# KinWaiCheuk/ReconVAT

Hardware: AMD Instinct MI355X
Metric: training audio-sec/sec (node) (higher is better)
Workload: dtype f32; 1 GPU; ReconVAT UNet_Onset VAT=True reconstruction=True, per-GPU B_l=8 + B_ul=8 segments of 327680 samples (640 frames x 229 mel), Adam+StepLR, fp32; parallelism=dp1, hipgraph=True, two_stream_schedule=True, kernel_plan_table=644fe159bb9eb70e, kernel_plan_mode=table, vat_nan_flag=0

## Files before the change

### include/reconvat_hip.h

```cpp
#ifndef RECONVAT_HIP_H
#define RECONVAT_HIP_H

#ifdef __cplusplus
extern "C" {
#endif

int rv_abi_version(void);
const char* rv_last_error(void);
const char* rv_source_digest(void);

int rv_melspec_lognorm_fwd(const float* audio, long audio_stride, int B, int nsamp, const float* window,
                           const float* twiddle, const int* mel_start, const int* mel_len, const float* mel_w, int mel_ld,
                           int n_mels, int hop, int do_log, int normalise, float* out, int T, void* workspace, void* stream);

long rv_cqt_workspace_bytes(int B, int nsamp, int n_items, int hop, int kernel_width);
int rv_cqt_lognorm_fwd(const float* audio, long audio_stride, int B, int nsamp, const float* w, long w_floats, const int* items,
                       int n_items, const int* groups, int n_groups, const float* scale, int n_bins, int kernel_width, int hop,
                       int do_log, int normalise, float* out, int T, void* workspace, long workspace_bytes, void* stream);

long rv_packed_weight_floats(int taps, int kdim, int ndim);
int rv_pack_weights(const float* w, float* out, int taps, int kdim, int ndim, long s_k, long s_n, int flip,
                    int scatter_cmid, int force_plain, void* stream);
long rv_pack_table_entry_bytes(void);
long rv_pack_table_fill(void* table_host, int i, const float* w, float* out, int taps, int kdim, int ndim, long s_k, long s_n,
                        int flip, int scatter_cmid, int force_plain);
int rv_pack_table_run(const void* table_dev, int count, long total_blocks, void* stream);
int rv_conv_fwd(int mode, const float* in, int in_ld, int B, int H, int W, int Cin, float* out, int out_ld, int Ho,
                int Wo, int Cout, const float* wpack, const float* bias, int accumulate, int algo, double* bn_sums,
                const float* bn_z, int bn_z_ld, const float* bn_coef, float bn_slope, void* stream);
long rv_conv_wgrad_workspace_bytes(int taps, int B, int Hv, int Ca, int Cb);
int rv_conv_wgrad_set_plan(int taps, int B, int Hv, int Ca, int Cb, int nw, int wgs);
int rv_conv_wgrad(int mode, const float* U, int u_ld, int Hu, int Wu, int Ca, const float* V, int v_ld, int Hv, int Wv,
                  int Cb, int B, float* dw, long s_a, long s_b, int flip, float* dbias, int accumulate, void* workspace,
                  long workspace_bytes, void* stream);
long rv_conv_wgrad_deferred(int mode, const float* U, int u_ld, int Hu, int Wu, int Ca, const float* V, int v_ld, int Hv, int Wv,
                            int Cb, int B, float* dw, long s_a, long s_b, int flip, float* dbias, void* workspace,
                            long workspace_bytes, void* entry_host, void* stream);
int rv_conv_wgrad_seg(int mode, int nseg, const float* const* U, const float* const* V, int u_ld, int Hu, int Wu, int Ca, int v_ld, int Hv,
                      int Wv, int Cb, int Bseg, float* dw, long s_a, long s_b, int flip, float* dbias, int accumulate, void* workspace,
                      long workspace_bytes, void* stream);
long rv_conv_wgrad_deferred_seg(int mode, int nseg, const float* const* U, const float* const* V, int u_ld, int Hu, int Wu, int Ca, int v_ld,
                                int Hv, int Wv, int Cb, int Bseg, float* dw, long s_a, long s_b, int flip, float* dbias, void* workspace,
                                long workspace_bytes, void* entry_host, void* stream);
long rv_wgrad_table_entry_bytes(void);
long rv_wgrad_table_finalize(void* table_host, int count);
int rv_wgrad_reduce_table(const void* table_dev, int count, long total_blocks, void* stream);


long rv_bn_workspace_bytes(int C);
int rv_bn_lrelu_fwd(const float* z, int z_ld, long P, int C, const float* gamma, const float* beta, float* running_mean,
                    float* running_var, long* num_batches_tracked, float momentum, float eps, int training, float slope,
                    const float* res, int res_ld, float* y, int y_ld, float* coef, void* workspace, int sums_ready,
                    void* stream);
int rv_bn_lrelu_fwd_skip(const float* z, int z_ld, long P, int C, const float* gamma, const float* beta, float* running_mean,
                         float* running_var, long* num_batches_tracked, float momentum, float eps, int training, float slope,
                         const float* x, int x_ld, int cin, const float* w, const float* b, int ksplit, float* y, int y_ld, float* coef,
                         void* workspace, int sums_ready, void* stream);
int rv_bn_running_update(float* running_mean, float* running_var, long* num_batches_tracked, const float* coef, int C,
                         float momentum, void* stream);
int rv_bn_running_update_table(const long* table, int nlayers, float momentum, void* stream);
int rv_bn_lrelu_bwd(const float* dy, int dy_ld, const float* z, int z_ld, long P, int C, const float* coef, float slope,
                    int frozen, float* dz, int dz_ld, float* dgamma, float* dbeta, int param_accumulate, void* workspace,
                    int sums_ready, void* stream);

long rv_gemm_splitk_workspace_bytes(int M, int N, int splitk, int batch);
long rv_gemm_splitk_ticket_bytes(int M, int N, int splitk, int batch);
int rv_gemm(const float* A, long sam, long sak, const float* B, long sbk, long sbn, float* C, long scm, long scn, float* C2,
            long sc2m, long sc2n, const float* bias, int M, int N, int K, int act, int accumulate, int splitk, int batch,
            long bsa, long bsb, long bsc, float* a_rowsum, void* splitk_ws, void* splitk_tickets, void* stream);
long rv_gemm_table_entry_bytes(void);
long rv_gemm_table_fill(void* entry_host, const float* A, long sam, long sak, const float* B, long sbk, long sbn, float* C, long scm,
                        long scn, const float* bias, int M, int N, int K, int splitk, int batch, long bsa, long bsb, long bsc,
                        float* a_rowsum, void* splitk_ws);
long rv_gemm_table_finalize(void* table_host, int count, long* fold_blocks);
int rv_gemm_table_run(const void* table_dev, int count, long total_blocks, long fold_blocks, int orientation, void* stream);
int rv_sigmoid_bwd(const float* g1, int ld1, const float* g2, int ld2, const float* y, int ldy, float* dz, int ldz, long M,
                   int N, void* stream);
int rv_colsum(const float* x, int ld, long M, int N, float* out, int accumulate, void* stream);
long rv_colsum_ordered_workspace_bytes(long M, int N);
int rv_colsum_ordered(const float* x, int ld, long M, int N, float* out, int accumulate, void* ws, void* stream);
int rv_sums_fold(const double* sums, int C, int c0, int n, float* out, int accumulate, void* stream);

// ... 82 lines not shown
```

### reconvat_amd/_lib.py

```python
import ctypes
import os

import torch

_HERE = os.path.dirname(os.path.abspath(__file__))
LIB_PATH = os.environ.get('RECONVAT_HIP_LIB') or os.path.join(_HERE, 'libreconvat_hip.so')

P = ctypes.c_void_p
U = ctypes.c_uint
I = ctypes.c_int
L = ctypes.c_long
F = ctypes.c_float

SIGNATURES = {
    'rv_abi_version': (I, []),
    'rv_last_error': (ctypes.c_char_p, []),
    'rv_source_digest': (ctypes.c_char_p, []),
    'rv_melspec_lognorm_fwd': (I, [P, L, I, I, P, P, P, P, P, I, I, I, I, I, P, I, P, P]),
    'rv_cqt_workspace_bytes': (L, [I, I, I, I, I]),
    'rv_cqt_lognorm_fwd': (I, [P, L, I, I, P, L, P, I, P, I, P, I, I, I, I, I, P, I, P, L, P]),
    'rv_packed_weight_floats': (L, [I, I, I]),
    'rv_pack_weights': (I, [P, P, I, I, I, L, L, I, I, I, P]),
    'rv_pack_table_entry_bytes': (L, []),
    'rv_pack_table_fill': (L, [P, I, P, P, I, I, I, L, L, I, I, I]),
    'rv_pack_table_run': (I, [P, I, L, P]),
    'rv_conv_fwd': (I, [I, P, I, I, I, I, I, P, I, I, I, I, P, P, I, I, P, P, I, P, F, P]),
    'rv_conv_wgrad_workspace_bytes': (L, [I, I, I, I, I]),
    'rv_conv_wgrad_set_plan': (I, [I, I, I, I, I, I, I]),
    'rv_conv_wgrad': (I, [I, P, I, I, I, I, P, I, I, I, I, I, P, L, L, I, P, I, P, L, P]),
    'rv_conv_wgrad_deferred': (L, [I, P, I, I, I, I, P, I, I, I, I, I, P, L, L, I, P, P, L, P, P]),
    'rv_conv_wgrad_seg': (I, [I, I, P, P, I, I, I, I, I, I, I, I, I, P, L, L, I, P, I, P, L, P]),
    'rv_conv_wgrad_deferred_seg': (L, [I, I, P, P, I, I, I, I, I, I, I, I, I, P, L, L, I, P, P, L, P, P]),
    'rv_wgrad_table_entry_bytes': (L, []),
    'rv_wgrad_table_finalize': (L, [P, I]),
    'rv_wgrad_reduce_table': (I, [P, I, L, P]),
    'rv_bn_workspace_bytes': (L, [I]),
    'rv_bn_lrelu_fwd': (I, [P, I, L, I, P, P, P, P, P, F, F, I, F, P, I, P, I, P, P, I, P]),
    'rv_bn_lrelu_fwd_skip': (I, [P, I, L, I, P, P, P, P, P, F, F, I, F, P, I, I, P, P, I, P, I, P, P, I, P]),
    'rv_bn_running_update': (I, [P, P, P, P, I, F, P]),
    'rv_bn_running_update_table': (I, [P, I, F, P]),
    'rv_bn_lrelu_bwd': (I, [P, I, P, I, L, I, P, F, I, P, I, P, P, I, P, I, P]),
    'rv_gemm_splitk_workspace_bytes': (L, [I, I, I, I]),
    'rv_gemm_splitk_ticket_bytes': (L, [I, I, I, I]),
    'rv_gemm': (I, [P, L, L, P, L, L, P, L, L, P, L, L, P, I, I, I, I, I, I, I, L, L, L, P, P, P, P]),
    'rv_gemm_table_entry_bytes': (L, []),
    'rv_gemm_table_fill': (L, [P, P, L, L, P, L, L, P, L, L, P, I, I, I, I, I, L, L, L, P, P]),
    'rv_gemm_table_finalize': (L, [P, I, P]),
    'rv_gemm_table_run': (I, [P, I, L, L, I, P]),
    'rv_sigmoid_bwd': (I, [P, I, P, I, P, I, P, I, L, I, P]),
    'rv_colsum': (I, [P, I, L, I, P, I, P]),
    'rv_colsum_ordered_workspace_bytes': (L, [L, I]),
    'rv_colsum_ordered': (I, [P, I, L, I, P, I, P, P]),
    'rv_sums_fold': (I, [P, I, I, I, P, I, P]),
    'rv_local_attn_fwd': (I, [P, P, P, L, P, P, P, I, I, I, I, P]),
    'rv_local_attn_bwd': (I, [P, P, P, P, L, P, P, P, P, P, L, P, I, I, I, I, P]),
    'rv_vat_perturb_fwd': (I, [P, P, L, I, F, F, P, P, P, P, P]),
    'rv_vat_perturb_bwd': (I, [P, P, P, L, I, F, F, P, P]),
    'rv_reduce_workspace_bytes': (L, [L]),
    'rv_reduce_mean': (I, [I, P, P, L, P, P, P, P]),
    'rv_loss_bwd': (I, [I, P, P, L, P, P, P]),
    'rv_adam_step': (I, [P, P, P, P, L, P, F, L, F, F, F, F, F, P, P]),
    'rv_counter_add': (I, [P, L, P, P]),
    'rv_clip_scale': (I, [P, L, P, F, P]),
    'rv_adamw_step': (I, [P, P, P, P, L, P, F, L, F, F, F, F, F, P, F, F, P, P, F, P]),
    'rv_swap_floats': (I, [P, P, L, P]),
    'rv_crop_segments': (I, [P, P, P, P, P, I, L, I, I, P, P, P, P, P, P]),
    'rv_crop_segments_shift': (I, [P, L, P, P, L, P, L, P, I, L, I, I, P, P, P, P, P, P]),
    'rv_fir_items': (I, [P, L, P, I, I, P, P, I, L, P, L, P]),
    'rv_resample_max_coeffs': (L, []),
    'rv_resample': (I, [P, I, L, I, L, P, I, I, I, I, P, I, L, L, P]),
    'rv_eval_workspace_bytes': (L, [L]),
    'rv_eval_decode': (I, [P, P, L, F, F, I, P, L, P, P, P, L, P]),
    'rv_eval_decode_clean': (I, [P, P, L, F, F, I, I, I, P, L, P, P, P, L, P]),
    'rv_eval_frame_counts': (I, [P, P, L, P, P, L, P]),
    'rv_eval_sweep_workspace_bytes': (L, [L, I, I]),
    'rv_eval_sweep': (I, [P, P, L, P, I, P, I, I, P, L, P, P, P, P, L, P]),
    'rv_eval_sweep_clean': (I, [P, P, L, P, I, P, I, I, I, I, P, L, P, P, P, P, L, P]),
    'rv_lstm_flag_bytes': (L, [I]),
    'rv_lstm_fwd': (I, [P, P, P, P, P, P, P, P, I, I, I, P]),
# ... 74 lines not shown
```

### reconvat_amd/csrc/conv.hip

```cpp
#include "conv_band.h"
#include <mutex>

struct PackArgs {
    const float* w;
    float* out;
    int taps, kdim, ndim;
    int R, ntile_n, nchunk;
    long s_k, s_n;
    int flip;
    int scatter_cmid;
    long total;
    long wino0;
};

__device__ __forceinline__ void pack_wino_elem(const PackArgs& a, long idx) {
    const int R = a.R;
    int r = (int)(idx % R);
    long t = idx / R;
    int lane = (int)(t % 64); t /= 64;
    int nt = (int)(t % a.ntile_n); t /= a.ntile_n;
    int c = (int)(t % a.nchunk);
    int xi = (int)(t / a.nchunk);
    int k = c * 4 * R + (lane >> 4) * R + r;
    int n = nt * 16 + (lane & 15);
// ... 174 lines not shown
#pragma unroll
            for (int n = 0; n < NT; ++n) {
                const int q = m * NT + n;
                if (q % KS != wave) continue;
                f32x4 sum = part[0][q][lane];
#pragma unroll
                for (int w = 1; w < KS; ++w) sum += part[w][q][lane];
                acc[m][n] = sum;
            }
    }
    f32x4 bv[NT];
#pragma unroll
    for (int n = 0; n < NT; ++n) {
        const int ncol = (nt0 + n) * 16 + 4 * g;
        const int cb = SCATTER ? ncol % a.Cout : ncol;
#pragma unroll
        for (int r = 0; r < 4; ++r) bv[n][r] = (a.bias && cb + r < a.Cout) ? a.bias[cb + r] : 0.f;
    }
#pragma unroll
    for (int m = 0; m < MT; ++m) {
        if (!pv[m]) continue;
#pragma unroll
        for (int n = 0; n < NT; ++n) {
            if (KS > 1 && (m * NT + n) % KS != wave) continue;
            const int ncol = (nt0 + n) * 16 + 4 * g;
            int co0;
            long opix;
            bool inside = true;
            if (SCATTER) {
                const int tap4 = ncol / a.Cout;
                co0 = ncol - tap4 * a.Cout;
                const int oy = py[m] * 2 + (tap4 >> 1), ox = px[m] * 2 + (tap4 & 1);
                inside = tap4 < 4 && oy < a.Ho && ox < a.Wo;
                opix = ((long)pb[m] * a.Ho + oy) * a.Wo + ox;
            } else {
                co0 = ncol;
                opix = (tile0 + m) * 16 + j;
            }
            if (!inside || co0 >= a.Cout) continue;
            float* o = a.out + opix * a.out_ld + co0;
            f32x4 v = acc[m][n] + bv[n];
            if (a.vec_store && co0 + 3 < a.Cout) {
                if (a.accumulate) {
                    f32x4 old = *reinterpret_cast<f32x4*>(o);
                    v += old;
                }
                *reinterpret_cast<f32x4*>(o) = v;
            } else {
#pragma unroll
                for (int r = 0; r < 4; ++r)
                    if (co0 + r < a.Cout) o[r] = a.accumulate ? o[r] + v[r] : v[r];
            }
        }
    }
}

__device__ __attribute__((aligned(16))) const float rv_zero_piece[256] = {0.f};

typedef short s16x4 __attribute__((ext_vector_type(4)));
typedef __bf16 bf16x2_t __attribute__((ext_vector_type(2)));
typedef __bf16 bf16x4_t __attribute__((ext_vector_type(4)));
__device__ __forceinline__ s16x4 to_bf16x4(const f32x4& v) {
    const bf16x2_t lo = __builtin_convertvector((f32x2){v[0], v[1]}, bf16x2_t);
    const bf16x2_t hi = __builtin_convertvector((f32x2){v[2], v[3]}, bf16x2_t);
    const bf16x4_t q = __builtin_shufflevector(lo, hi, 0, 1, 2, 3);
    return __builtin_bit_cast(s16x4, q);
}

template <int R, int NT, int MTW, int NW, bool BF = false>
__global__ __launch_bounds__(NW * 64) void conv3x3_lds_k(ConvLdsArgs aa) {
    static_assert(!BF || R == 4, "the bf16 path needs 16-channel chunks");
    constexpr int NTHR = NW * 64;
    typedef typename VecR<R>::T vec;
    constexpr int KC = 4 * R;
    constexpr int Q = R;
    constexpr int PPI = 64 / Q;
    constexpr int LPF = 16 * R;
    constexpr int FPI = 64 / LPF;
    constexpr int WFLOATS = 9 * NT * 64 * R;
    const ConvArgs& a = aa.c;
    extern __shared__ __attribute__((aligned(16))) float smem[];
    const int tid = threadIdx.x, lane = tid & 63;
    const int wave = __builtin_amdgcn_readfirstlane(tid >> 6);
    const int j = lane & 15, g = lane >> 4;
    const int W = a.W, H = a.H, W2 = W + 2, TH = aa.TH;
    const int nrow = TH + 2;
    const int xfloats = nrow * W2 * KC;
    if (ABL(aa) & 32) return;
    const int vid = aa.xcd ? xcd_remap(blockIdx.x, gridDim.x) : blockIdx.x;
    const int grp = vid / aa.nsplit, split = vid - grp * aa.nsplit;
    const int nt0 = split * NT;
    const int nbuf = aa.nbuf;
    float* xs0 = smem;
    float* ws0 = smem + nbuf * xfloats;
    const int band_lo = grp * aa.bands_per_wg;
    const int band_hi = min(band_lo + aa.bands_per_wg, aa.total_bands);
    if (band_lo >= band_hi) return;
    const int nchunk = a.nchunk;
    const int nunits = (band_hi - band_lo) * nchunk;
    const int ipr = (W + PPI - 1) / PPI;

    constexpr int TXF = 4;
    constexpr int NWF = (9 * NT + FPI - 1) / FPI;
    constexpr int TW = (NWF + NW - 1) / NW;
    const int nx = nrow * ipr;
    int xs_row[TXF], xs_ldst[TXF];
// ... 2047 lines not shown
        ent = tab[lo];
    }
    __syncthreads();
    const long block = (long)blockIdx.x - ent.block0;
#ifdef RV_ABLATION
    if (plain) {
        ent.a.accumulate = 0;
        if (ent.vec4 && ent.el == 64) wgrad_reduce_body_v4<64, false>(ent.a, block, sh);
        else if (ent.vec4 && ent.el == 16) wgrad_reduce_body_v4<16, false>(ent.a, block, sh);
        else if (ent.el == 64) wgrad_reduce_body<64, false>(ent.a, block, sh);
        else if (ent.el == 16) wgrad_reduce_body<16, false>(ent.a, block, sh);
        else wgrad_reduce_body<4, false>(ent.a, block, sh);
        return;
    }
#endif
    if (ent.vec4 && ent.el == 1024) wgrad_reduce_body_v4<1024, true>(ent.a, block, sh);
    else if (ent.vec4 && ent.el == 64) wgrad_reduce_body_v4<64, true>(ent.a, block, sh);
    else if (ent.vec4 && ent.el == 16) wgrad_reduce_body_v4<16, true>(ent.a, block, sh);
    else if (ent.el == 64) wgrad_reduce_body<64, true>(ent.a, block, sh);
    else if (ent.el == 16) wgrad_reduce_body<16, true>(ent.a, block, sh);
    else wgrad_reduce_body<4, true>(ent.a, block, sh);
}

template <int KH, int KW, int S, int P, int R, bool SC>
static int launch_conv_rt(const ConvArgs& a, int NT, int MT, hipStream_t st, bool ksplit = false) {
    const long ntiles = (a.npix + 15) / 16;
    if (ksplit) {
        if constexpr (R == 4 && !(KH == 3)) {
#define RV_CASEK(nt, mt)                                                                         \
    if (NT == nt && MT == mt) {                                                                  \
        dim3 grid(cdiv(ntiles, mt), a.ntile_n / nt);                                             \
        hipLaunchKernelGGL((conv_mfma_k<KH, KW, S, P, R, nt, mt, SC, 4>), grid, dim3(256), 0, st, a); \
        return RV_OK;                                                                            \
    }
            RV_CASEK(1, 1) RV_CASEK(1, 2) RV_CASEK(2, 1) RV_CASEK(2, 2) RV_CASEK(1, 4) RV_CASEK(4, 1)
#undef RV_CASEK
        }
        return RV_EUNSUPPORTED;
    }
#define RV_CASE(nt, mt)                                                                          \
    if (NT == nt && MT == mt) {                                                                  \
        dim3 grid(cdiv(ntiles, 4 * mt), a.ntile_n / nt);                                         \
        hipLaunchKernelGGL((conv_mfma_k<KH, KW, S, P, R, nt, mt, SC>), grid, dim3(256), 0, st, a); \
        return RV_OK;                                                                            \
    }
    RV_CASE(1, 1) RV_CASE(1, 2) RV_CASE(1, 4)
    RV_CASE(2, 1) RV_CASE(2, 2) RV_CASE(2, 4)
    RV_CASE(3, 1) RV_CASE(3, 2) RV_CASE(3, 4)
    RV_CASE(4, 1) RV_CASE(4, 2) RV_CASE(4, 4)
#undef RV_CASE
    return RV_EUNSUPPORTED;
}

static void choose_tiles(long ntiles, int ntile_n, int* NT, int* MT) {
    static const int nts[4] = {4, 3, 2, 1};
    static const int mts[3] = {4, 2, 1};
    int best_nt = 1, best_mt = 1;
    long best_score = -1;
    for (int a = 0; a < 4; ++a) {
        int nt = nts[a];
        if (ntile_n % nt) continue;
        for (int b = 0; b < 3; ++b) {
            int mt = mts[b];
            long waves = ((ntiles + mt - 1) / mt) * (ntile_n / nt);
            long reuse = (long)(nt * mt * 100) / (nt + mt);
            long fill = waves >= 2048 ? 100 : (waves * 100) / 2048;
            long score = reuse * fill;
            if (score > best_score) { best_score = score; best_nt = nt; best_mt = mt; }
        }
    }
    *NT = best_nt; *MT = best_mt;
}

static size_t conv3x3_lds_bytes(int R, int NT, int TH, int W, int nchunk, int nbuf = 2) {
    return ((size_t)nbuf * (TH + 2) * (W + 2) * 4 * R + (size_t)(nchunk > 1 ? nbuf : 1) * 9 * NT * 64 * R) * sizeof(float);
}

template <int R, int NW, bool BF = false>
static int launch_conv3x3_lds_r(const ConvArgs& a, int NT, int MTW, int TH, int wgs_per_cu, hipStream_t st) {
    ConvLdsArgs aa;
    aa.c = a; aa.TH = TH;
    dim3 grid(band_grid(aa, NT, 256 * wgs_per_cu)), blk(NW * 64);
    static const int nbuf_env = getenv("RV_CONV_NBUF") ? atoi(getenv("RV_CONV_NBUF")) : 0;
    aa.nbuf = 2;
    if (nbuf_env == 3 && conv3x3_lds_bytes(R, NT, TH, a.W, a.nchunk, 3) <= (size_t)(wgs_per_cu > 1 ? 76 : 150) * 1024) aa.nbuf = 3;
    aa.ablate = getenv("RV_ABLATE") ? atoi(getenv("RV_ABLATE")) : 0;
    static const int skew_env = getenv("RV_CONV_SKEW") ? atoi(getenv("RV_CONV_SKEW")) : 1;
    aa.skew = (aa.nbuf == 3 && NW >= 8) ? skew_env : 0;
    const size_t lds = conv3x3_lds_bytes(R, NT, TH, a.W, a.nchunk, aa.nbuf);
#define RV_L3(nt, mt)                                                                              \
    if (NT == nt && MTW == mt) {                                                                  \
        auto kern = conv3x3_lds_k<R, nt, mt, NW, BF>;                                             \
         \
        static std::once_flag attr_once;                                                          \
        std::call_once(attr_once, [&] {                                                           \
             \
            if (hipFuncSetAttribute((const void*)kern, hipFuncAttributeMaxDynamicSharedMemorySize, 156 * 1024) != hipSuccess) \
                (void)hipGetLastError();                                                          \
        });                                                                                       \
        hipLaunchKernelGGL(kern, grid, blk, lds, st, aa);                                         \
        return RV_OK;                                                                             \
    }
    if constexpr (NW == 12) {
        RV_L3(1, 3) RV_L3(2, 3) RV_L3(3, 3) RV_L3(4, 3)
        RV_L3(1, 5) RV_L3(2, 5) RV_L3(1, 6) RV_L3(2, 6)
        RV_L3(1, 1) RV_L3(2, 1) RV_L3(4, 1) RV_L3(1, 2) RV_L3(2, 2) RV_L3(4, 2) RV_L3(1, 4) RV_L3(2, 4)
// ... 149 lines not shown
    }
    return RV_OK;
}

int rv_pack_weights(const float* w, float* out, int taps, int kdim, int ndim, long s_k, long s_n, int flip,
                    int scatter_cmid, int force_plain, void* stream) {
    PackArgs a;
    const int rc = pack_args_make(a, w, out, taps, kdim, ndim, s_k, s_n, flip, scatter_cmid, force_plain);
    if (rc != RV_OK) return rc;
    hipStream_t st = (hipStream_t)stream;
    if (a.R == 0) hipLaunchKernelGGL(pack_plain_k, dim3(cdiv(a.total, 256)), dim3(256), 0, st, a);
    else hipLaunchKernelGGL(pack_frag_k, dim3(cdiv(a.total, 256)), dim3(256), 0, st, a);
    RV_LAUNCH_CHECK("rv_pack_weights");
    return RV_OK;
}

long rv_pack_table_entry_bytes(void) { return (long)sizeof(PackEntry); }

long rv_pack_table_fill(void* table, int i, const float* w, float* out, int taps, int kdim, int ndim, long s_k, long s_n,
                        int flip, int scatter_cmid, int force_plain) {
    PackEntry* tab = (PackEntry*)table;
    if (pack_args_make(tab[i].a, w, out, taps, kdim, ndim, s_k, s_n, flip, scatter_cmid, force_plain) != RV_OK) return -1;
    tab[i].block0 = i == 0 ? 0 : tab[i - 1].block0 + cdiv(tab[i - 1].a.total, 256);
    return tab[i].block0 + cdiv(tab[i].a.total, 256);
}

int rv_pack_table_run(const void* table_dev, int count, long total_blocks, void* stream) {
    RV_CHECK_ARG(count > 0 && total_blocks > 0 && total_blocks < (1L << 31), "rv_pack_table_run: empty or oversized table");
    hipLaunchKernelGGL(pack_table_k, dim3((unsigned)total_blocks), dim3(256), 0, (hipStream_t)stream,
                       (const PackEntry*)table_dev, count);
    RV_LAUNCH_CHECK("rv_pack_table_run");
    return RV_OK;
}

struct BnFuse { double* sums; const float* z; int z_ld; const float* coef; float slope; };
static int conv_fwd_impl(int mode, const float* in, int in_ld, int B, int H, int W, int Cin, float* out, int out_ld, int Ho,
                         int Wo, int Cout, const float* wpack, const float* bias, int accumulate, int algo, const BnFuse& bn,
                         bool* sums_done, hipStream_t st);

int rv_conv_fwd(int mode, const float* in, int in_ld, int B, int H, int W, int Cin, float* out, int out_ld, int Ho,
                int Wo, int Cout, const float* wpack, const float* bias, int accumulate, int algo, double* bn_sums,
                const float* bn_z, int bn_z_ld, const float* bn_coef, float bn_slope, void* stream) {
    hipStream_t st = (hipStream_t)stream;
    bool sums_done = false;
    RV_CHECK_ARG(!bn_z || (bn_sums && bn_coef), "rv_conv_fwd: bn_z needs bn_sums and bn_coef");
    const BnFuse bn = {bn_sums, bn_z, bn_z_ld, bn_coef, bn_slope};
    const int rc = conv_fwd_impl(mode, in, in_ld, B, H, W, Cin, out, out_ld, Ho, Wo, Cout, wpack, bias, accumulate, algo,
                                 bn, &sums_done, st);
    if (rc != RV_OK || !bn_sums || sums_done) return rc;
    if (bn_z) return rv_internal_bn_bwd_stats(out, out_ld, bn_z, bn_z_ld, (long)B * Ho * Wo, Cout, bn_coef, bn_slope, bn_sums, st);
    return rv_internal_bn_stats(out, out_ld, (long)B * Ho * Wo, Cout, bn_sums, st);
}

static int conv_fwd_impl(int mode, const float* in, int in_ld, int B, int H, int W, int Cin, float* out, int out_ld, int Ho,
                         int Wo, int Cout, const float* wpack, const float* bias, int accumulate, int algo, const BnFuse& bn,
                         bool* sums_done, hipStream_t st) {
    double* bn_sums = bn.sums;
    RV_CHECK_ARG(mode >= 0 && mode <= 3, "rv_conv_fwd: bad mode %d", mode);
    if (mode == 0 || mode == 1) RV_CHECK_ARG(Ho == H && Wo == W, "rv_conv_fwd: same-size conv needs Ho==H, Wo==W");
    if (mode == 2) RV_CHECK_ARG(Ho == H / 2 && Wo == W / 2, "rv_conv_fwd: down conv needs Ho=H/2, Wo=W/2");
    if (mode == 3)
        RV_CHECK_ARG(Ho >= 2 * H && Ho <= 2 * H + 1 && Wo >= 2 * W && Wo <= 2 * W + 1,
                     "rv_conv_fwd: up conv needs 2H<=Ho<=2H+1 (got H=%d Ho=%d W=%d Wo=%d)", H, Ho, W, Wo);
    const int R = frag_R(Cin);
    const bool small = (R == 0) || (Cout <= 2 && mode != 3);
    if (small) {
        SmallArgs s;
        s.in = in; s.in_ld = in_ld; s.H = H; s.W = W; s.out = out; s.out_ld = out_ld; s.Ho = Ho; s.Wo = Wo;
        s.B = B; s.wplain = wpack; s.bias = bias; s.npix = (long)B * Ho * Wo; s.accumulate = accumulate;
        s.fd_plane = fastdiv_make((unsigned)(Ho * Wo)); s.fd_wo = fastdiv_make((unsigned)Wo);
        const int tpp = Cout / small_cpt(Cin, Cout, mode == 0 ? 9 : 1);
        RV_CHECK_ARG(s.npix * tpp < (1L << 31), "rv_conv_fwd: more than 2^31 outputs");
        s.bn_sums = (Cout >= 4 && !bn.z) ? bn_sums : nullptr;
        if (s.bn_sums) *sums_done = true;
        long nblk = cdiv(s.npix * tpp, 256);
        const long cap = s.bn_sums ? 1024 : 4096;
        if (nblk > cap) nblk = cap;
        dim3 grid((unsigned)nblk), blk(256);
#define RV_SMALL(ci, co, kh, kw, ss, pp)                                                          \
    if (Cin == ci && Cout == co) {                                                               \
        hipLaunchKernelGGL((conv_small_k<ci, co, kh, kw, ss, pp>), grid, blk, 0, st, s);         \
        RV_LAUNCH_CHECK("conv_small");                                                           \
        return RV_OK;                                                                            \
    }
#define RV_NARROW(ci, co)                                                                         \
    if (mode == 0 && Cin == ci && Cout == co && (in_ld & 3) == 0 && ((((uintptr_t)in) & 15) == 0)) { \
        RV_CHECK_ARG(s.npix < (1L << 28), "rv_conv_fwd: more than 2^28 pixels");                \
        static const int nrows_env = getenv("RV_NARROW_ROWS") ? atoi(getenv("RV_NARROW_ROWS")) : 16;   \
        s.rows = nrows_env;                                                                      \
        const long nb = (long)B * cdiv(H, s.rows) * cdiv(W, 256 / (ci / 4));                     \
        hipLaunchKernelGGL((conv_narrow_out_k<ci, co>), dim3((unsigned)nb), blk, 0, st, s);      \
        RV_LAUNCH_CHECK("conv_narrow_out");                                                      \
        return RV_OK;                                                                            \
    }
        RV_NARROW(16, 1) RV_NARROW(8, 2) RV_NARROW(8, 1)
#undef RV_NARROW
        static const int cin1_env = getenv("RV_CONV_CIN1") ? atoi(getenv("RV_CONV_CIN1")) : 1;
        const bool cin12 = mode == 0 && ((Cin == 1 && (Cout == 16 || Cout == 8)) || (Cin == 2 && Cout == 8 && (in_ld & 1) == 0 && ((((uintptr_t)in) & 7) == 0)));
        const bool bz_ok = !bn.z || ((bn.z_ld & 3) == 0 && ((((uintptr_t)bn.z) & 15) == 0) && ((((uintptr_t)bn.coef) & 15) == 0));
        if (cin1_env && cin12 && bz_ok && (!bias || ((((uintptr_t)bias) & 15) == 0))) {
            s.rows = 16;
            s.bn_z = bn.z; s.bn_z_ld = bn.z_ld; s.bn_coef = bn.coef; s.bn_slope = bn.slope;
            if (bn.z) { s.bn_sums = bn_sums; *sums_done = true; }
            const long nb = (long)B * cdiv(H, s.rows) * cdiv(W, 1024 / Cout);
            if (Cin == 1 && Cout == 16) hipLaunchKernelGGL((conv_cin12_k<1, 16>), dim3((unsigned)nb), blk, 0, st, s);
            else if (Cin == 1) hipLaunchKernelGGL((conv_cin12_k<1, 8>), dim3((unsigned)nb), blk, 0, st, s);
            else hipLaunchKernelGGL((conv_cin12_k<2, 8>), dim3((unsigned)nb), blk, 0, st, s);
            RV_LAUNCH_CHECK("conv_cin12");
            return RV_OK;
        }
        if (mode == 0) {
            RV_SMALL(1, 16, 3, 3, 1, 1) RV_SMALL(16, 1, 3, 3, 1, 1)
            RV_SMALL(8, 2, 3, 3, 1, 1)  RV_SMALL(2, 8, 3, 3, 1, 1)
            RV_SMALL(8, 1, 3, 3, 1, 1)  RV_SMALL(1, 8, 3, 3, 1, 1)
            RV_SMALL(1, 48, 3, 3, 1, 1) RV_SMALL(48, 1, 3, 3, 1, 1)
        } else if (mode == 1) {
            RV_SMALL(1, 16, 1, 1, 1, 0) RV_SMALL(16, 1, 1, 1, 1, 0)
        }
#undef RV_SMALL
        rv_set_error("rv_conv_fwd: no small-channel kernel for mode %d Cin=%d Cout=%d", mode, Cin, Cout);
        return RV_EUNSUPPORTED;
    }
    ConvArgs a;
    a.in = in; a.in_ld = in_ld; a.H = H; a.W = W; a.out = out; a.out_ld = out_ld; a.Ho = Ho; a.Wo = Wo;
    a.B = B; a.Cin = Cin; a.Cout = Cout; a.wpack = wpack; a.bias = bias; a.bn_sums = bn_sums;
    a.bn_z = bn.z; a.bn_z_ld = bn.z_ld; a.bn_coef = bn.coef; a.bn_slope = bn.slope;
    a.nchunk = Cin / (4 * R);
    a.accumulate = accumulate;
    a.vec_store = ((out_ld & 3) == 0) && ((((uintptr_t)out) & 15) == 0);
    RV_CHECK_ARG((in_ld % R) == 0 && ((((uintptr_t)in) & (4 * R - 1)) == 0), "rv_conv_fwd: input not %d-byte aligned", 4 * R);
    if (mode == 3) {
        RV_CHECK_ARG(Cout % 16 == 0, "rv_conv_fwd: scatter conv needs Cout %% 16 == 0");
        a.ntile_n = 4 * Cout / 16;
        a.Ph = H + (Ho - 2 * H); a.Pw = W + (Wo - 2 * W);
    } else {
        a.ntile_n = (Cout + 15) / 16;
        a.Ph = Ho; a.Pw = Wo;
    }
    a.npix = (long)B * a.Ph * a.Pw;
    a.fd_pw = fastdiv_make((unsigned)a.Pw); a.fd_plane = fastdiv_make((unsigned)(a.Ph * a.Pw)); a.fd_w = fastdiv_make((unsigned)W);
    RV_CHECK_ARG(a.npix < (1L << 31), "rv_conv_fwd: more than 2^31 pixels");
    const bool bf = ((algo >> 20) & 1) && mode == 0 && R == 4;
    algo &= ~(1 << 20);
    const int fam = (algo >> 8) & 15, f_nt = (algo >> 4) & 15, f_mt = algo & 15, f_th = (algo >> 12) & 255;
    if (fam == 6 || fam == 10 || fam == 12) {
        if (mode != 0 || R != 4) { rv_set_error("rv_conv_fwd: the Winograd kernel needs a 3x3 conv with Cin %% 16 == 0"); return RV_EUNSUPPORTED; }
        const int rcw = fam == 6 ? launch_conv3x3_wino<8>(a, f_nt, f_mt, f_th, st)
                                 : (fam == 10 ? launch_conv3x3_wino<8, true>(a, f_nt, f_mt, f_th, st) : launch_conv3x3_wino<12, true>(a, f_nt, f_mt, f_th, st));
        if (rcw != RV_OK) { rv_set_error("rv_conv_fwd: forced Winograd tile NT=%d MTW=%d TH=%d does not fit", f_nt, f_mt, f_th); return rcw; }
        RV_LAUNCH_CHECK("rv_conv_fwd(winograd)");
        *sums_done = true;
        return RV_OK;
    }
    if (fam == 14) {
        if (mode != 0 || R != 4) { rv_set_error("rv_conv_fwd: the Winograd kernel needs a 3x3 conv with Cin %% 16 == 0"); return RV_EUNSUPPORTED; }
        const int rcw = launch_conv3x3_wino<4, true>(a, f_nt, f_mt, f_th, st, (size_t)78 * 1024, 512);
        if (rcw != RV_OK) { rv_set_error("rv_conv_fwd: forced half-CU Winograd tile NT=%d MTW=%d TH=%d does not fit", f_nt, f_mt, f_th); return rcw; }
        RV_LAUNCH_CHECK("rv_conv_fwd(winograd, half CU)");
        *sums_done = true;
        return RV_OK;
    }
    if (fam == 8 || fam == 9 || fam == 11 || fam == 13) {
        if (mode != 0 || R != 4) { rv_set_error("rv_conv_fwd: the Winograd kernel needs a 3x3 conv with Cin %% 16 == 0"); return RV_EUNSUPPORTED; }
        const int rcw = rv_launch_conv3x3_wino2(a, f_nt, f_mt, fam == 13 ? 12 : ((fam == 8 || fam == 9) ? 8 : 4), (fam == 9 || fam == 13) ? 1 : 0, f_th, st);
        if (rcw != RV_OK) { rv_set_error("rv_conv_fwd: forced pipelined Winograd tile NT=%d MTW=%d TH=%d does not fit", f_nt, f_mt, f_th); return rcw; }
        RV_LAUNCH_CHECK("rv_conv_fwd(winograd, pipelined)");
        *sums_done = true;
        return RV_OK;
    }
    if (mode == 0 && algo != 1 && fam != 1 && fam != 5) {
        const bool forced = (fam >= 2 && fam <= 4) || fam == 7;
        int rc3 = forced ? launch_conv3x3_lds(a, R, st, f_nt, f_mt, fam == 7 ? 12 : (fam == 4 ? 16 : (fam == 3 ? 8 : 4)), f_th, bf)
                         : launch_conv3x3_lds(a, R, st, 0, 0, 4, 0, bf);
        if (rc3 == RV_OK) { RV_LAUNCH_CHECK("rv_conv_fwd(lds)"); *sums_done = true; return RV_OK; }
        if (forced) { rv_set_error("rv_conv_fwd: forced LDS tile NT=%d MTW=%d does not fit", f_nt, f_mt); return RV_EUNSUPPORTED; }
    }
    int NT, MT;
    choose_tiles((a.npix + 15) / 16, a.ntile_n, &NT, &MT);
    const bool ksplit = fam == 5;
    if (ksplit) {
        if (mode == 0 || R != 4 || f_nt < 1 || a.ntile_n % f_nt || a.nchunk * (mode == 2 ? 4 : 1) < 4) {
            rv_set_error("rv_conv_fwd: forced split-K direct tile NT=%d MT=%d invalid here", f_nt, f_mt);
            return RV_EUNSUPPORTED;
        }
        NT = f_nt; MT = f_mt;
    }
    if (fam == 1) {
        if (f_nt < 1 || a.ntile_n % f_nt || !(f_mt == 1 || f_mt == 2 || f_mt == 4) || f_nt > 4) {
            rv_set_error("rv_conv_fwd: forced direct tile NT=%d MT=%d invalid", f_nt, f_mt);
            return RV_EUNSUPPORTED;
        }
        NT = f_nt; MT = f_mt;
    }
    int rc = RV_EUNSUPPORTED;
    if (R == 4) {
        if (mode == 0) rc = launch_conv_rt<3, 3, 1, 1, 4, false>(a, NT, MT, st);
        else if (mode == 1) rc = launch_conv_rt<1, 1, 1, 0, 4, false>(a, NT, MT, st, ksplit);
        else if (mode == 2) rc = launch_conv_rt<2, 2, 2, 0, 4, false>(a, NT, MT, st, ksplit);
        else rc = launch_conv_rt<1, 1, 1, 0, 4, true>(a, NT, MT, st, ksplit);
    } else {
        if (mode == 0) rc = launch_conv_rt<3, 3, 1, 1, 2, false>(a, NT, MT, st);
        else if (mode == 1) rc = launch_conv_rt<1, 1, 1, 0, 2, false>(a, NT, MT, st);
        else if (mode == 2) rc = launch_conv_rt<2, 2, 2, 0, 2, false>(a, NT, MT, st);
        else rc = launch_conv_rt<1, 1, 1, 0, 2, true>(a, NT, MT, st);
    }
    if (rc != RV_OK) { rv_set_error("rv_conv_fwd: no kernel instance for NT=%d MT=%d", NT, MT); return rc; }
    RV_LAUNCH_CHECK("rv_conv_fwd");
    return RV_OK;
}

struct WgradPlan { bool small; int TA, TB, nga, ngb, rows_per_wave, nparts, nw; bool wino; };

struct WgradTune { int taps, B, Hv, Ca, Cb, nw, wgs; };
static WgradTune g_wgrad_tune[256];
static int g_wgrad_ntune = 0;
static const WgradTune* wgrad_tuned(int taps, int B, int Hv, int Ca, int Cb) {
    for (int i = 0; i < g_wgrad_ntune; ++i) {
        const WgradTune& t = g_wgrad_tune[i];
        if (t.taps == taps && t.B == B && t.Hv == Hv && t.Ca == Ca && t.Cb == Cb) return &t;
    }
    return nullptr;
}

static WgradPlan wgrad_plan(int taps, int B, int Hv, int Ca, int Cb) {
    WgradPlan p;
    p.nw = 0;
    p.wino = false;
    const int nrows = B * Hv;
    p.small = (Ca * Cb * taps <= 144) && (Ca < 8 || Cb < 8);
    if (p.small) {
        p.TA = p.TB = p.nga = p.ngb = 1; p.rows_per_wave = 0;
        { static int np = getenv("RV_WGS_NPARTS") ? atoi(getenv("RV_WGS_NPARTS")) : 4096; p.nparts = nrows < np ? nrows : np; }
        return p;
    }
    long best = -1;
    p.TA = p.TB = 1;
    for (int ta = 2; ta >= 1; --ta)
        for (int tb = 2; tb >= 1; --tb) {
            const long padded = (long)cdiv(Ca, ta * 16) * ta * cdiv(Cb, tb * 16) * tb;
            if (best < 0 || padded < best) { best = padded; p.TA = ta; p.TB = tb; }
        }
    p.nga = cdiv(Ca, p.TA * 16); p.ngb = cdiv(Cb, p.TB * 16);
    static int want_total = 0;
    if (!want_total) { const char* e = getenv("RV_WGRAD_WGS"); want_total = e ? atoi(e) : 256; }
    int total = want_total;
// ... 308 lines not shown
```

### reconvat_amd/tuning.py

```python
import operator
import os
import sys

from . import plans

ALGO_BF16 = 1 << 20
FAMILIES = {
    1: ('conv_mfma_k', 4, False, False),
    2: ('conv3x3_lds_k', 4, False, False),
    3: ('conv3x3_lds_k', 8, False, False),
    4: ('conv3x3_lds_k', 16, False, False),
    5: ('conv_mfma_k', 4, False, True),
    6: ('conv3x3_wino_k', 8, True, False),
    7: ('conv3x3_lds_k', 12, False, False),
    8: ('conv3x3_wino2_k', 8, True, False),
    9: ('conv3x3_wino2_k', 8, True, False),
    10: ('conv3x3_wino_k', 8, True, False),
    11: ('conv3x3_wino2_k', 4, True, False),
    12: ('conv3x3_wino_k', 12, True, False),
    13: ('conv3x3_wino2_k', 12, True, False),
    14: ('conv3x3_wino_k', 4, True, False),
}
WINOGRAD_FAMILIES = tuple(f for f, v in FAMILIES.items() if v[2])
KSPLIT_FAMILIES = tuple(f for f, v in FAMILIES.items() if v[3])
LDS_WAVES = {f: v[1] for f, v in FAMILIES.items() if v[0] == 'conv3x3_lds_k'}

_algo_cache = {}
_algo_unchecked = set()
_tune_us = {}
_tune_top = {}
_gemm_splitk = {}
_wgrad_tuned = set()
_wgrad_plans = {}
_wgrad_owner = {}


def encode(fam, nt, mt, th=0):
    return th << 12 | fam << 8 | nt << 4 | mt


def decode(algo):
    return (algo >> 8) & 15, (algo >> 4) & 15, algo & 15, (algo >> 12) & 255, bool(algo & ALGO_BF16)


def bf16_form(algo):
    if decode(algo)[0] in WINOGRAD_FAMILIES:
        algo = 0
    return algo if algo == 1 or decode(algo)[0] == 1 else algo | ALGO_BF16


_WINOGRAD_TILES = ((6, ((1, 1),), False), (10, ((1, 1), (2, 1)), False), (12, ((1, 1),), False),
                   (8, ((1, 1),), True), (9, ((1, 1), (2, 1), (1, 2)), True), (11, ((1, 2), (2, 1)), True), (13, ((1, 1),), True))


def conv_candidates(mode, h, w, cin, cout, *, winograd=True, wino2=True, families=None):
    ntile_n = (4 * cout if mode == 3 else cout + 15) // 16
    cands = [1, 2] if mode == 0 else [0]
    for nt in (1, 2, 3, 4):
        if ntile_n % nt:
# ... 136 lines not shown
```

Baseline: 16570 audio-s/s.

## Add persistent streaming conv kernel with register-resident weights and software-pipelined loads

Adds a persistent-wave forward conv kernel for 1x1, strided 2x2 and transposed-scatter modes. It keeps all weight fragments in registers, walks pixel tiles with a grid stride, and prefetches input tiles several slots ahead of the MFMA compute. It is enabled by default for eligible convs with at least 131072 pixels, and can be forced or forbidden through algo bits. The aim is to cut repeated weight loads and hide input load latency on large, low-channel convs. The cost is high register pressure and limited occupancy.

```diff
diff --git a/include/reconvat_hip.h b/include/reconvat_hip.h
--- a/include/reconvat_hip.h
+++ b/include/reconvat_hip.h
@@ -28,6 +28,7 @@
 int rv_conv_fwd(int mode, const float* in, int in_ld, int B, int H, int W, int Cin, float* out, int out_ld, int Ho,
                 int Wo, int Cout, const float* wpack, const float* bias, int accumulate, int algo, double* bn_sums,
                 const float* bn_z, int bn_z_ld, const float* bn_coef, float bn_slope, void* stream);
+int rv_conv_fwd_form(int mode, int B, int H, int W, int Cin, int Ho, int Wo, int Cout, int algo);
 long rv_conv_wgrad_workspace_bytes(int taps, int B, int Hv, int Ca, int Cb);
 int rv_conv_wgrad_set_plan(int taps, int B, int Hv, int Ca, int Cb, int nw, int wgs);
 int rv_conv_wgrad(int mode, const float* U, int u_ld, int Hu, int Wu, int Ca, const float* V, int v_ld, int Hv, int Wv,
diff --git a/reconvat_amd/_lib.py b/reconvat_amd/_lib.py
--- a/reconvat_amd/_lib.py
+++ b/reconvat_amd/_lib.py
@@ -25,6 +25,7 @@
     'rv_pack_table_fill': (L, [P, I, P, P, I, I, I, L, L, I, I, I]),
     'rv_pack_table_run': (I, [P, I, L, P]),
     'rv_conv_fwd': (I, [I, P, I, I, I, I, I, P, I, I, I, I, P, P, I, I, P, P, I, P, F, P]),
+    'rv_conv_fwd_form': (I, [I, I, I, I, I, I, I, I, I]),
     'rv_conv_wgrad_workspace_bytes': (L, [I, I, I, I, I]),
     'rv_conv_wgrad_set_plan': (I, [I, I, I, I, I, I, I]),
     'rv_conv_wgrad': (I, [I, P, I, I, I, I, P, I, I, I, I, I, P, L, L, I, P, I, P, L, P]),
diff --git a/reconvat_amd/csrc/conv.hip b/reconvat_amd/csrc/conv.hip
--- a/reconvat_amd/csrc/conv.hip
+++ b/reconvat_amd/csrc/conv.hip
@@ -250,6 +250,177 @@
                     if (co0 + r < a.Cout) o[r] = a.accumulate ? o[r] + v[r] : v[r];
             }
         }
+    }
+}
+
+struct ConvStreamArgs {
+    ConvArgs c;
+    long ntiles;
+    int step_b, step_y, step_x;
+};
+
+template <int MODE, int NS> struct StreamDepth {
+    static constexpr int KIB = MODE == 3 ? 4 : 8;
+    static constexpr int AHEAD = NS >= KIB + 1 ? 1 : (NS >= KIB / 2 ? 2 : (KIB + NS - 1) / NS);
+};
+
+template <int MODE, int NC, int NTN, int KS>
+__global__ __launch_bounds__(256) void conv_stream_k(ConvStreamArgs sa) {
+    constexpr int TAPS = MODE == 2 ? 4 : 1, NS = TAPS * NC;
+    constexpr int AHEAD = StreamDepth<MODE, NS>::AHEAD, NB = AHEAD + 1;
+    constexpr int NPT = MODE == 3 ? NTN / 4 : NTN;
+    static_assert(MODE != 3 || NTN % 4 == 0, "the scatter form has four taps of Cout / 16 n-tiles");
+    static_assert(NS * NTN <= 16, "the weights must fit in 64 registers");
+    static_assert(KS == 1 || (KS == 4 && NS >= 4), "split chains need four steps");
+    const ConvArgs& a = sa.c;
+    const int lane = threadIdx.x & 63, wave = threadIdx.x >> 6;
+    const int j = lane & 15, g = lane >> 4;
+    const long gw = (long)xcd_remap(blockIdx.x, gridDim.x) * 4 + wave;
+    const long nwaves = (long)gridDim.x * 4;
+    if (gw >= sa.ntiles) return;
+
+    f32x4 wf[NS][NTN];
+#pragma unroll
+    for (int s = 0; s < NS; ++s)
+#pragma unroll
+        for (int n = 0; n < NTN; ++n) wf[s][n] = *reinterpret_cast<const f32x4*>(a.wpack + ((long)(s * NTN + n) * 64 + lane) * 4);
+    f32x4 bv[NPT];
+#pragma unroll
+    for (int n = 0; n < NPT; ++n) {
+        const int cb = n * 16 + 4 * g;
+#pragma unroll
+        for (int r = 0; r < 4; ++r) bv[n][r] = (a.bias && cb + r < a.Cout) ? a.bias[cb + r] : 0.f;
+    }
+    const long o_row = (long)a.Wo * a.out_ld;
+
+    const int stride_px = (int)nwaves * 16;
+    long lp = gw * 16 + j;
+    int lb = 0, ly = 0, lx = 0;
+    if (MODE != 1) {
+        const unsigned pp = lp < a.npix ? (unsigned)lp : 0u;
+        lb = (int)fastdiv(pp, a.fd_plane);
+        const unsigned rem = pp - (unsigned)lb * (unsigned)(a.Ph * a.Pw);
+        ly = (int)fastdiv(rem, a.fd_pw);
+        lx = (int)rem - ly * a.Pw;
+    }
+    const long tap_x = a.in_ld, tap_y = (long)a.W * a.in_ld;
+
+    f32x4 xf[NB][NS];
+    int s_fl[NB];
+    long s_out[NB];
+
+    auto load_slot = [&](auto slot) {
+        constexpr int i = decltype(slot)::value;
+        const bool pv = lp < a.npix;
+        bool ok = pv;
+        long ioff, ooff;
+        if (MODE == 1) {
+            ioff = lp * a.in_ld;
+            ooff = lp * a.out_ld;
+        } else if (MODE == 2) {
+            ioff = (((long)lb * a.H + 2 * ly) * a.W + 2 * lx) * a.in_ld;
+            ooff = lp * a.out_ld;
+        } else {
+            ok = pv && ly < a.H && lx < a.W;
+            ioff = (((long)lb * a.H + ly) * a.W + lx) * a.in_ld;
+            ooff = (((long)lb * a.Ho + 2 * ly) * a.Wo + 2 * lx) * a.out_ld;
+        }
+        s_fl[i] = (pv ? 1 : 0) | ((MODE == 3 && 2 * ly + 1 < a.Ho) ? 2 : 0) | ((MODE == 3 && 2 * lx + 1 < a.Wo) ? 4 : 0);
+        s_out[i] = ooff;
+        const float* src = a.in + ioff + g * 4;
+#pragma unroll
+        for (int t = 0; t < TAPS; ++t)
+#pragma unroll
+            for (int c = 0; c < NC; ++c) {
+                f32x4 v = (f32x4){0.f, 0.f, 0.f, 0.f};
+                if (ok) v = *reinterpret_cast<const f32x4*>(src + (t >> 1) * tap_y + (t & 1) * tap_x + c * 16);
+                xf[i][t * NC + c] = v;
+            }
+        lp += stride_px;
+        if (MODE != 1) {
+            lx += sa.step_x;
+            if (lx >= a.Pw) { lx -= a.Pw; ++ly; }
+            ly += sa.step_y;
+            if (ly >= a.Ph) { ly -= a.Ph; ++lb; }
+            lb += sa.step_b;
+        }
+    };
+
+    auto compute_slot = [&](auto slot) {
+        constexpr int i = decltype(slot)::value;
+        f32x4 acc[NTN];
+        if constexpr (KS == 1) {
+#pragma unroll
+            for (int n = 0; n < NTN; ++n) acc[n] = (f32x4){0.f, 0.f, 0.f, 0.f};
+#pragma unroll
+            for (int s = 0; s < NS; ++s)
+#pragma unroll
+                for (int r = 0; r < 4; ++r)
+#pragma unroll
+                    for (int n = 0; n < NTN; ++n) acc[n] = __builtin_amdgcn_mfma_f32_16x16x4f32(wf[s][n][r], xf[i][s][r], acc[n], 0, 0, 0);
+        } else {
+            f32x4 part[KS][NTN];
+#pragma unroll
+            for (int w = 0; w < KS; ++w)
+#pragma unroll
+                for (int n = 0; n < NTN; ++n) part[w][n] = (f32x4){0.f, 0.f, 0.f, 0.f};
+#pragma unroll
+            for (int s = 0; s < NS; ++s) {
+                int w = 0;
+#pragma unroll
+                for (int q = 1; q < KS; ++q)
+                    if (s >= (q * NS) / KS) w = q;
+#pragma unroll
+                for (int r = 0; r < 4; ++r)
+#pragma unroll
+                    for (int n = 0; n < NTN; ++n) part[w][n] = __builtin_amdgcn_mfma_f32_16x16x4f32(wf[s][n][r], xf[i][s][r], part[w][n], 0, 0, 0);
+            }
+#pragma unroll
+            for (int n = 0; n < NTN; ++n) {
+                f32x4 sum = part[0][n];
+#pragma unroll
+                for (int w = 1; w < KS; ++w) sum += part[w][n];
+                acc[n] = sum;
+            }
+        }
+        if (!(s_fl[i] & 1)) return;
+#pragma unroll
+        for (int n = 0; n < NTN; ++n) {
+            const int co0 = (n % NPT) * 16 + 4 * g;
+            long opix = 0;
+            bool inside = true;
+            if (MODE == 3) {
+                const int tap4 = n / NPT;
+                inside = ((tap4 >> 1) == 0 || (s_fl[i] & 2)) && ((tap4 & 1) == 0 || (s_fl[i] & 4));
+                opix = (tap4 >> 1) * o_row + (tap4 & 1) * (long)a.out_ld;
+            }
+            if (!inside || co0 >= a.Cout) continue;
+            float* o = a.out + s_out[i] + opix + co0;
+            f32x4 v = acc[n] + bv[n % NPT];
+            if (a.vec_store && co0 + 3 < a.Cout) {
+                if (a.accumulate) {
+                    f32x4 old = *reinterpret_cast<f32x4*>(o);
+                    v += old;
+                }
+                *reinterpret_cast<f32x4*>(o) = v;
+            } else {
+#pragma unroll
+                for (int r = 0; r < 4; ++r)
+                    if (co0 + r < a.Cout) o[r] = a.accumulate ? o[r] + v[r] : v[r];
+            }
+        }
+    };
+
+    sfor<0, AHEAD>([&](auto k) { load_slot(k); });
+    for (long t = gw; t < sa.ntiles;) {
+        sfor<0, NB>([&](auto k) {
+            constexpr int i = decltype(k)::value;
+            if (t < sa.ntiles) {
+                load_slot(std::integral_constant<int, (i + AHEAD) % NB>{});
+                compute_slot(k);
+                t += nwaves;
+            }
+        });
     }
 }
 
@@ -2403,6 +2574,68 @@
     return RV_EUNSUPPORTED;
 }
 
+#define RV_ALGO_STREAM (1 << 21)
+#define RV_ALGO_TILE (1 << 22)
+static const long RV_CONV_STREAM_MIN_PIXELS = 131072;
+static int conv_stream_env(const char* name, int dflt) { return getenv(name) ? atoi(getenv(name)) : dflt; }
+static const int g_conv_stream_env = conv_stream_env("RV_CONV_STREAM", 1);
+static const int g_conv_stream_wgs_env = conv_stream_env("RV_CONV_STREAM_WGS", 0);
+
+static bool conv_stream_eligible(int mode, int R, const ConvArgs& a) {
+    return mode >= 1 && mode <= 3 && R == 4 && (mode == 2 ? 4 : 1) * a.nchunk * a.ntile_n <= 16;
+}
+
+static int conv_stream_form(int mode, int R, const ConvArgs& a, int algo) {
+    const bool s = (algo & RV_ALGO_STREAM) != 0, t = (algo & RV_ALGO_TILE) != 0;
+    const int fam = (algo >> 8) & 15;
+    const bool ok = conv_stream_eligible(mode, R, a) && (fam == 0 || fam == 1 || fam == 5);
+    if (s && t) return -1;
+    if (s) return ok ? 1 : -1;
+    if (t) return 0;
+    return (g_conv_stream_env && ok && a.npix >= RV_CONV_STREAM_MIN_PIXELS) ? 1 : 0;
+}
+
+template <int MODE, int KS, int NC = 1, int NTN = 1>
+static int launch_conv_stream_rt(const ConvStreamArgs& sa, int wg_cap, hipStream_t st) {
+    constexpr int TAPS = MODE == 2 ? 4 : 1, NS = TAPS * NC;
+    if constexpr (NS * NTN > 16) {
+        if constexpr (NTN == 1) return RV_EUNSUPPORTED;
+        else return launch_conv_stream_rt<MODE, KS, NC + 1, 1>(sa, wg_cap, st);
+    } else {
+        if constexpr (!(MODE == 3 && NTN % 4 != 0) && !(KS == 4 && NS < 4)) {
+            if (sa.c.nchunk == NC && sa.c.ntile_n == NTN) {
+                static const int resident = [] {
+                    int n = 0;
+                    return hipOccupancyMaxActiveBlocksPerMultiprocessor(&n, conv_stream_k<MODE, NC, NTN, KS>, 256, 0) == hipSuccess && n > 0 ? n : 1;
+                }();
+                int per_cu = g_conv_stream_wgs_env > 0 ? g_conv_stream_wgs_env : (MODE == 3 ? 4 : 2);
+                if (per_cu > resident) per_cu = resident;
+                const long trips = cdiv(sa.ntiles, 4 * 256L * per_cu);
+                long wgs = cdiv(sa.ntiles, 4 * trips);
+                if (wg_cap > 0 && wgs > wg_cap) wgs = wg_cap;
+                ConvStreamArgs s = sa;
+                const long stride = wgs * 4 * 16, plane = (long)s.c.Ph * s.c.Pw;
+                s.step_b = (int)(stride / plane);
+                s.step_y = (int)((stride % plane) / s.c.Pw);
+                s.step_x = (int)((stride % plane) % s.c.Pw);
+                hipLaunchKernelGGL((conv_stream_k<MODE, NC, NTN, KS>), dim3((unsigned)wgs), dim3(256), 0, st, s);
+                return RV_OK;
+            }
+        }
+        return launch_conv_stream_rt<MODE, KS, NC, NTN + 1>(sa, wg_cap, st);
+    }
+}
+
+static int launch_conv_stream(int mode, const ConvArgs& a, bool ksplit, int wg_cap, hipStream_t st) {
+    ConvStreamArgs sa;
+    sa.c = a;
+    sa.ntiles = (a.npix + 15) / 16;
+    sa.step_b = sa.step_y = sa.step_x = 0;
+    if (mode == 1) return ksplit ? launch_conv_stream_rt<1, 4>(sa, wg_cap, st) : launch_conv_stream_rt<1, 1>(sa, wg_cap, st);
+    if (mode == 2) return ksplit ? launch_conv_stream_rt<2, 4>(sa, wg_cap, st) : launch_conv_stream_rt<2, 1>(sa, wg_cap, st);
+    return ksplit ? launch_conv_stream_rt<3, 4>(sa, wg_cap, st) : launch_conv_stream_rt<3, 1>(sa, wg_cap, st);
+}
+
 static void choose_tiles(long ntiles, int ntile_n, int* NT, int* MT) {
     static const int nts[4] = {4, 3, 2, 1};
     static const int mts[3] = {4, 2, 1};
@@ -2658,6 +2891,16 @@
     return rv_internal_bn_stats(out, out_ld, (long)B * Ho * Wo, Cout, bn_sums, st);
 }
 
+int rv_conv_fwd_form(int mode, int B, int H, int W, int Cin, int Ho, int Wo, int Cout, int algo) {
+    const int R = frag_R(Cin);
+    if (mode < 0 || mode > 3 || R == 0 || (Cout <= 2 && mode != 3)) return (algo & RV_ALGO_STREAM) ? -1 : 0;
+    ConvArgs a;
+    a.nchunk = Cin / (4 * R);
+    a.ntile_n = mode == 3 ? 4 * Cout / 16 : (Cout + 15) / 16;
+    a.npix = mode == 3 ? (long)B * (H + (Ho - 2 * H)) * (W + (Wo - 2 * W)) : (long)B * Ho * Wo;
+    return conv_stream_form(mode, R, a, algo);
+}
+
 static int conv_fwd_impl(int mode, const float* in, int in_ld, int B, int H, int W, int Cin, float* out, int out_ld, int Ho,
                          int Wo, int Cout, const float* wpack, const float* bias, int accumulate, int algo, const BnFuse& bn,
                          bool* sums_done, hipStream_t st) {
@@ -2671,6 +2914,7 @@
     const int R = frag_R(Cin);
     const bool small = (R == 0) || (Cout <= 2 && mode != 3);
     if (small) {
+        if (algo & RV_ALGO_STREAM) { rv_set_error("rv_conv_fwd: the streaming form needs Cin %% 16 == 0 (Cin=%d Cout=%d)", Cin, Cout); return RV_EUNSUPPORTED; }
         SmallArgs s;
         s.in = in; s.in_ld = in_ld; s.H = H; s.W = W; s.out = out; s.out_ld = out_ld; s.Ho = Ho; s.Wo = Wo;
         s.B = B; s.wplain = wpack; s.bias = bias; s.npix = (long)B * Ho * Wo; s.accumulate = accumulate;
@@ -2747,7 +2991,16 @@
     a.fd_pw = fastdiv_make((unsigned)a.Pw); a.fd_plane = fastdiv_make((unsigned)(a.Ph * a.Pw)); a.fd_w = fastdiv_make((unsigned)W);
     RV_CHECK_ARG(a.npix < (1L << 31), "rv_conv_fwd: more than 2^31 pixels");
     const bool bf = ((algo >> 20) & 1) && mode == 0 && R == 4;
-    algo &= ~(1 << 20);
+    const int form = conv_stream_form(mode, R, a, algo);
+    if (form < 0) {
+        rv_set_error((algo & RV_ALGO_STREAM) && (algo & RV_ALGO_TILE)
+                         ? "rv_conv_fwd: RV_ALGO_STREAM and RV_ALGO_TILE exclude each other"
+                         : "rv_conv_fwd: the streaming form needs mode 1-3, Cin %% 16 == 0, at most 16 weight fragments and family 0, 1 or 5 (mode %d Cin=%d Cout=%d)",
+                     mode, Cin, Cout);
+        return RV_EUNSUPPORTED;
+    }
+    const int stream_cap = (algo & RV_ALGO_STREAM) ? (algo >> 12) & 255 : 0;
+    algo &= ~((1 << 20) | RV_ALGO_STREAM | RV_ALGO_TILE);
     const int fam = (algo >> 8) & 15, f_nt = (algo >> 4) & 15, f_mt = algo & 15, f_th = (algo >> 12) & 255;
     if (fam == 6 || fam == 10 || fam == 12) {
         if (mode != 0 || R != 4) { rv_set_error("rv_conv_fwd: the Winograd kernel needs a 3x3 conv with Cin %% 16 == 0"); return RV_EUNSUPPORTED; }
@@ -2797,6 +3050,14 @@
             return RV_EUNSUPPORTED;
         }
         NT = f_nt; MT = f_mt;
+    }
+    if (form == 1) {
+        if (launch_conv_stream(mode, a, ksplit, stream_cap, st) != RV_OK) {
+            rv_set_error("rv_conv_fwd: no streaming instance for nchunk=%d ntile_n=%d", a.nchunk, a.ntile_n);
+            return RV_EUNSUPPORTED;
+        }
+        RV_LAUNCH_CHECK("rv_conv_fwd(stream)");
+        return RV_OK;
     }
     int rc = RV_EUNSUPPORTED;
     if (R == 4) {
diff --git a/reconvat_amd/tuning.py b/reconvat_amd/tuning.py
--- a/reconvat_amd/tuning.py
+++ b/reconvat_amd/tuning.py
@@ -5,6 +5,8 @@
 from . import plans
 
 ALGO_BF16 = 1 << 20
+ALGO_STREAM = 1 << 21
+ALGO_TILE = 1 << 22
 FAMILIES = {
     1: ('conv_mfma_k', 4, False, False),
     2: ('conv3x3_lds_k', 4, False, False),
```

After: 16620 audio-s/s, median of 6. About the same (+0.3%).
